# biscuitzb/COEB-SLAM

Hardware: AMD Instinct MI355X
Metric: frames/sec ORB extract+match @640x480/1000 kp; 1/2/4/8 GPU + %HBM roofline (higher is better)
Workload: dtype u8; 1 GPU; 640x480, 8-level pyramid, 1000 kp, extract + Hamming match to prev frame (BASELINE configs[1]); width=640, height=480, nfeatures=1000, nlevels=8, halo_frames_per_rank=1, pipelines_per_gpu=3, streams_per_gpu=1, ranks=single, parallelism=frame-sharded x1 (no collectives), hw_queues=4, side_stream=own, side_stream_created=with the context

## Files before the change

### coeb-slam_amd/csrc/coeb_extract.hip

```cpp
#include <type_traits>
#include <cmath>
#include <hip/hip_runtime.h>

#include "coeb_internal.hpp"

namespace {

constexpr int kThreads = 256;
constexpr int kWaves = kThreads / 64;

__device__ __forceinline__ int lane_id() { return __lane_id(); }
__device__ __forceinline__ int wave_id() { return __builtin_amdgcn_readfirstlane(threadIdx.x >> 6); }
__device__ __forceinline__ void wave_sync_lds()
{
    __builtin_amdgcn_fence(__ATOMIC_RELEASE, "wavefront");
    __builtin_amdgcn_wave_barrier();
    __builtin_amdgcn_fence(__ATOMIC_ACQUIRE, "wavefront");
}
typedef unsigned int u32x4 __attribute__((ext_vector_type(4)));

__device__ __forceinline__ uint64_t lanemask_lt() { return (1ull << lane_id()) - 1ull; }

__device__ __forceinline__ int wave_sum(int v)
{
// ... 81 lines not shown
        const int rx = (int)xmin, ry = (int)ymin, rw = (int)(xmax - xmin), rh = (int)(ymax - ymin);
        const float area_box = (xmax - xmin) * (ymax - ymin);
        bool mark = false;
        unsigned long long nin = 0;
        for (int t = t0; t < t1; t++) {
            const int px = (int)tm[2 * t], py = (int)tm[2 * t + 1];
            const bool in = px >= 0 && px < W && py >= 0 && py < H && px >= rx && px < rx + rw &&
                            py >= ry && py < ry + rh;
            if (in) nin++;
            if ((float)(nin * 10000ull) > area_box) { mark = true; break; }
        }
        const int bf = b.blurf ? b.blurf[bi] : 0;
        if (mark || (bf == 1 && nin > 0)) {
            area = area + area_box;
            const int x0 = max((int)xmin, 0), x1 = min((int)xmax, W);
            const int y0 = max((int)ymin, 0), y1 = min((int)ymax, H);
            if (x1 > x0 && y1 > y0) {
                if (m.nrect < COEB_MAXBOX) {
                    m.rect[m.nrect][0] = x0; m.rect[m.nrect][1] = y0;
                    m.rect[m.nrect][2] = x1; m.rect[m.nrect][3] = y1;
                    m.nrect++;
                } else {
                    atomicOr(b.err, 1);
                }
            }
        }
    }
    m.area_flag = area > 200000.f ? 1 : 0;
    b.dyn[f] = m;
}

typedef unsigned short us2 __attribute__((ext_vector_type(2)));
typedef float f32x2 __attribute__((ext_vector_type(2)));

__device__ __forceinline__ us2 as_us2(uint32_t v) { return __builtin_bit_cast(us2, v); }
__device__ __forceinline__ uint32_t as_u32(us2 v) { return __builtin_bit_cast(uint32_t, v); }
__device__ __forceinline__ us2 pk2(int lo, int hi) { us2 r; r.x = (unsigned short)lo; r.y = (unsigned short)hi; return r; }

__device__ __forceinline__ int byte_of(uint32_t w0, uint32_t w1, uint32_t w2, int o)
{
    const uint32_t w = o < 4 ? w0 : (o < 8 ? w1 : w2);
    return (int)((w >> ((o & 3) * 8)) & 0xFFu);
}

__device__ __forceinline__ uint32_t vresize_g(uint32_t g0, uint32_t g1, uint32_t b0s, uint32_t b1s)
{
    const uint32_t m0 = __umulhi(g0 & 0xFFFF00u, b0s & 0xFFFFFFu);
    const uint32_t m1 = __umulhi(g1 & 0xFFFF00u, b1s & 0xFFFFFFu);
    return (m0 + m1 + 2u) >> 2;
}

constexpr int PT_W = 128, PT_H = 32;

void pyr_tile_lds(int sw, int sh, int dw, int dh, int* tsw, int* tsh)
{
    const int span = (int)std::ceil(127.0 * sw / dw) + 2 + 15;
    *tsw = 16 * ((span + 15) / 16 + 1);
    *tsh = (int)std::ceil(31.0 * sh / dh) + 4;
}

int resize_simd_end(int w)
{
    int x = w >= 16 ? (w / 16) * 16 : 0;
    while (x < w - 4) x += 4;
    return x;
}

__device__ __forceinline__ uint32_t vresize_exact(uint32_t g0, uint32_t g1, uint32_t b0s, uint32_t b1s)
{
    const uint32_t v = __umul24(g0 >> 4, b0s >> 8) + __umul24(g1 >> 4, b1s >> 8) + (1u << 21);
    return min(v >> 22, 255u);
}

__global__ __launch_bounds__(kThreads) void k_pyr_level(const uint8_t* __restrict__ src, int64_t src_fs, int sp,
                                                        int sw, int sh, uint8_t* __restrict__ dst, int64_t dst_fs,
                                                        int dp, int dw, int dh, const int* __restrict__ tab, int xmax,
                                                        int xs, int tsw, int tsh)
{
    extern __shared__ __attribute__((aligned(16))) uint8_t s_src[];
    const int f = blockIdx.z;
    const int ox = blockIdx.x * PT_W, oy = blockIdx.y * PT_H;
    const int* xofs = tab;
    const int* alpha = tab + dw;
    const int* yofs = tab + 2 * dw;
    const int* beta = tab + 2 * dw + dh;
    const int ex = min(ox + PT_W, dw) - 1, ey = min(oy + PT_H, dh) - 1;
    const int sx1 = min(xofs[ex] + 1, sw - 1);
    const int sy0 = max(yofs[oy], 0), sy1 = min(max(yofs[ey] + 1, 0), sh - 1);
    const int nrows = sy1 - sy0 + 1;
    const uint8_t* S = src + (int64_t)f * src_fs;
    const int tid = threadIdx.x;
    int sx0;
    const bool vec = ((sp | (int)reinterpret_cast<uintptr_t>(S)) & 15) == 0;
    if (vec && ((sx1 - (xofs[ox] & ~15)) >> 4) + 1 <= tsw / 16 && nrows <= tsh) {
        sx0 = xofs[ox] & ~15;
        const int nch = ((sx1 - sx0) >> 4) + 1;
        const int rstep = kThreads / nch;
        const int r = tid / nch, k = tid - r * nch;
        if (r < rstep) {
            const uint4* base = reinterpret_cast<const uint4*>(S + (int64_t)sy0 * sp + sx0) + k;
            const int pw = sp >> 4;
            uint4 q0 = base[min(r, nrows - 1) * pw];
            uint4 q1 = base[min(r + rstep, nrows - 1) * pw];
            uint4 q2 = base[min(r + 2 * rstep, nrows - 1) * pw];
            if (r < nrows) *reinterpret_cast<uint4*>(s_src + r * tsw + 16 * k) = q0;
            if (r + rstep < nrows) *reinterpret_cast<uint4*>(s_src + (r + rstep) * tsw + 16 * k) = q1;
            if (r + 2 * rstep < nrows) *reinterpret_cast<uint4*>(s_src + (r + 2 * rstep) * tsw + 16 * k) = q2;
            for (int rr = r + 3 * rstep; rr < nrows; rr += rstep)
                *reinterpret_cast<uint4*>(s_src + rr * tsw + 16 * k) = base[rr * pw];
        }
    } else if ((sp & 3) == 0) {
        sx0 = xofs[ox] & ~3;
        const int nwords = (sx1 - sx0) / 4 + 1;
        for (int i = tid; i < nwords * nrows; i += kThreads) {
            const int r = i / nwords, k = i - r * nwords;
            *reinterpret_cast<uint32_t*>(s_src + r * tsw + 4 * k) =
                *reinterpret_cast<const uint32_t*>(S + (int64_t)(sy0 + r) * sp + sx0 + 4 * k);
        }
    } else {
        sx0 = xofs[ox];
        const int nb = sx1 - sx0 + 1;
        for (int i = tid; i < nb * nrows; i += kThreads) {
            const int r = i / nb, k = i - r * nb;
            s_src[r * tsw + k] = S[(int64_t)(sy0 + r) * sp + sx0 + k];
        }
    }
    __syncthreads();
    const int cx = ox + (threadIdx.x & 31) * 4, cy = oy + (threadIdx.x >> 5) * 4;
    if (cx >= dw) return;
    const int nk = min(4, dw - cx);
    int lx[4], a0[4], a1[4];
#pragma unroll
    for (int k = 0; k < 4; k++) {
        const int d = min(cx + k, dw - 1);
        const int sx = xofs[d];
        const int a = alpha[d];
        a0[k] = ((int)(short)(a & 0xFFFF)) << 4;
        a1[k] = (a >> 16) << 4;
        if (d >= xmax) { a0[k] = 2048 << 4; a1[k] = 0; }
        lx[k] = sx - sx0;
    }
#pragma unroll
    for (int r = 0; r < 4; r++) {
        const int dy = cy + r;
        if (dy >= dh) break;
        const int q0 = yofs[dy];
        const int r0 = (q0 >= 0 ? (q0 < sh ? q0 : sh - 1) : 0) - sy0;
        const int r1 = (q0 + 1 >= 0 ? (q0 + 1 < sh ? q0 + 1 : sh - 1) : 0) - sy0;
        const int bb = beta[dy];
        const uint32_t b0s = (uint32_t)((int)(short)(bb & 0xFFFF)) << 8, b1s = (uint32_t)(bb >> 16) << 8;
        const uint8_t* R0 = s_src + __mul24(r0, tsw);
        const uint8_t* R1 = s_src + __mul24(r1, tsw);
        uint32_t word = 0;
#pragma unroll
        for (int k = 0; k < 4; k++) {
            const int g0 = __mul24((int)R0[lx[k]], a0[k]) + __mul24((int)R0[lx[k] + 1], a1[k]);
            const int g1 = __mul24((int)R1[lx[k]], a0[k]) + __mul24((int)R1[lx[k] + 1], a1[k]);
            const uint32_t v = cx + k < xs ? vresize_g((uint32_t)g0, (uint32_t)g1, b0s, b1s)
                                           : vresize_exact((uint32_t)g0, (uint32_t)g1, b0s, b1s);
            word |= v << (8 * k);
        }
        uint8_t* D = dst + (int64_t)f * dst_fs + (int64_t)dy * dp + cx;
        if (nk == 4 && (dp & 3) == 0) *reinterpret_cast<uint32_t*>(D) = word;
        else for (int k = 0; k < nk; k++) D[k] = (uint8_t)(word >> (8 * k));
    }
}

constexpr int PR_ROWS = 8, PR_COLS = 128;

__device__ __forceinline__ uint32_t ld_u32(const uint8_t* p) { return *reinterpret_cast<const uint32_t*>(p); }

template <bool kTail, bool kEdge>
__device__ __forceinline__ void pyr_rows_out(const uint32_t (&w)[PR_ROWS][4], const uint32_t (&sel)[2],
                                             const uint32_t (&coef)[2], const int4* __restrict__ yrow,
                                             __amdgpu_buffer_rsrc_t rd, int oy, int dh, uint32_t cx, int dw, int xs)
{
#pragma unroll
    for (int r = 0; r < PR_ROWS; r++) {
        const int dy = oy + r;
        if (dy >= dh) break;
        const int4 yr = yrow[dy];
        const uint32_t bb = (uint32_t)yr.z;
        const uint32_t b0 = bb & 0xFFFFu, b1 = bb >> 16;
        const uint32_t b0s = (bb << 12) & 0xFFF000u, b1s = (bb >> 4) & 0xFFF000u;
        uint32_t v[2];
#pragma unroll
        for (int k = 0; k < 2; k++) {
            const uint32_t h0 = __builtin_amdgcn_udot2(as_us2(__builtin_amdgcn_perm(w[r][1], w[r][0], sel[k])),
                                                       as_us2(coef[k]), 0u, false);
            const uint32_t h1 = __builtin_amdgcn_udot2(as_us2(__builtin_amdgcn_perm(w[r][3], w[r][2], sel[k])),
                                                       as_us2(coef[k]), 0u, false);
            v[k] = (__umulhi(h0 & 0xFFFF0u, b0s) + __umulhi(h1 & 0xFFFF0u, b1s) + 2u) >> 2;
            if (kTail && (int)cx + k >= xs)
                v[k] = min((__umul24(h0, b0) + __umul24(h1, b1) + (1u << 21)) >> 22, 255u);
        }
        const uint32_t pr = v[0] | (v[1] << 8);
        if (!kEdge) {
            __builtin_amdgcn_raw_buffer_store_b16((uint16_t)pr, rd, cx, yr.w, 0);
        } else {
            if ((int)cx + 1 < dw) __builtin_amdgcn_raw_buffer_store_b16((uint16_t)pr, rd, cx, yr.w, 0);
            else if ((int)cx < dw) __builtin_amdgcn_raw_buffer_store_b8((uint8_t)pr, rd, cx, yr.w, 0);
        }
    }
}

__global__ __launch_bounds__(kThreads) void k_pyr_rows(const uint8_t* __restrict__ src, int64_t src_fs, int sp,
                                                       int sh, uint8_t* __restrict__ dst, int64_t dst_fs, int dp,
                                                       int dw, int dh, const int* __restrict__ tab, int xmax, int xs,
                                                       const int4* __restrict__ yrow)
{
    const int f = blockIdx.z;
    const int oy = (blockIdx.y * kWaves + wave_id()) * PR_ROWS;
    if (oy >= dh) return;
    const int lane = lane_id();
    const int ox = blockIdx.x * PR_COLS;
    const uint32_t cx = (uint32_t)(ox + 2 * lane);
    const int* xofs = tab;
    const int* alpha = tab + dw;
    uint32_t sel[2], coef[2];
    const int d0 = min((int)cx, dw - 1);
    const uint32_t wb = (uint32_t)(xofs[d0] & ~3);
    const uint32_t wb1 = (uint32_t)min((int)wb + 4, sp - 4);
#pragma unroll
    for (int k = 0; k < 2; k++) {
        const int d = min((int)cx + k, dw - 1);
        const int o = xofs[d] - (int)wb;
        const int a = alpha[d];
        const uint32_t a0 = d >= xmax ? 2048u : (uint32_t)(a & 0xFFFF), a1 = d >= xmax ? 0u : (uint32_t)a >> 16;
        coef[k] = a0 | (a1 << 16);
        sel[k] = (uint32_t)o | 0x0c00u | ((uint32_t)(o + 1) << 16) | 0x0c000000u;
    }
    const __amdgpu_buffer_rsrc_t rs =
        __builtin_amdgcn_make_buffer_rsrc((void*)(src + (int64_t)f * src_fs), 0, 0x7fffffff, 0x00020000);
    const __amdgpu_buffer_rsrc_t rd =
        __builtin_amdgcn_make_buffer_rsrc((void*)(dst + (int64_t)f * dst_fs), 0, 0x7fffffff, 0x00020000);
    uint32_t w[PR_ROWS][4];
#pragma unroll
    for (int r = 0; r < PR_ROWS; r++) {
        const int4 yr = yrow[min(oy + r, dh - 1)];
        w[r][0] = __builtin_amdgcn_raw_buffer_load_b32(rs, wb, yr.x, 0);
        w[r][1] = __builtin_amdgcn_raw_buffer_load_b32(rs, wb1, yr.x, 0);
        w[r][2] = __builtin_amdgcn_raw_buffer_load_b32(rs, wb, yr.y, 0);
        w[r][3] = __builtin_amdgcn_raw_buffer_load_b32(rs, wb1, yr.y, 0);
    }
    (void)dp;
    const bool edge = ox + PR_COLS > dw - 1;
    if (ox + PR_COLS > xs) {
        if (edge) pyr_rows_out<true, true>(w, sel, coef, yrow, rd, oy, dh, cx, dw, xs);
        else pyr_rows_out<true, false>(w, sel, coef, yrow, rd, oy, dh, cx, dw, xs);
    } else {
        if (edge) pyr_rows_out<false, true>(w, sel, coef, yrow, rd, oy, dh, cx, dw, xs);
        else pyr_rows_out<false, false>(w, sel, coef, yrow, rd, oy, dh, cx, dw, xs);
    }
}

constexpr int kBlurCols = 56;

__device__ __forceinline__ int reflect101(int p, int len)
{
    if (len == 1) return 0;
    while (p < 0 || p >= len) p = p < 0 ? -p : 2 * len - p - 2;
    return p;
}

struct BlurWork {
    int L;
    int item0, item1;
    int item_off[COEB_MAXL + 1];
    int nstrips[COEB_MAXL];
    int bh[COEB_MAXL];
    int nquads[COEB_MAXL];
    int brows;
};


template <bool kRemap = true>
__device__ __forceinline__ int2 block_xy()
{
    const int gx = gridDim.x;
    if (!kRemap) return make_int2(blockIdx.x, blockIdx.y);
    const int n = gx * gridDim.y, p = blockIdx.x + gx * blockIdx.y;
    const int q = n >> 3, r = n & 7, x = p & 7, k = p >> 3;
    const int lg = x * q + min(x, r) + k;
    return make_int2(lg % gx, lg / gx);
}

__device__ __forceinline__ uint32_t dpp_shr1(uint32_t v)
{
    return (uint32_t)__builtin_amdgcn_mov_dpp((int)v, 0x111, 0xf, 0xf, false);
}
__device__ __forceinline__ uint32_t dpp_shl1(uint32_t v)
{
    return (uint32_t)__builtin_amdgcn_mov_dpp((int)v, 0x101, 0xf, 0xf, false);
}

__device__ __forceinline__ int reflect_row(int r, int h)
{
    int rr = r < 0 ? -r : r;
    rr = rr >= h ? 2 * h - 2 - rr : rr;
    return rr < 0 ? 0 : rr;
}

constexpr int kBlurQuad = 4 * kBlurCols;
static_assert(kBlurQuad % 16 == 0, "a wave item must cover whole 16-column tiles");

__global__ __launch_bounds__(kThreads) void k_blur_rows(const Plan* __restrict__ P, ExtractBufs b, BlurWork bw)
{
    __shared__ __attribute__((aligned(16))) uint8_t s_tile[kWaves][8 * kBlurQuad];
    const int2 bxy = block_xy();
    const int f = bxy.y;
    const int item = bw.item0 + bxy.x * kWaves + wave_id();
    if (item >= bw.item1) return;
    int l = 0;
    while (l + 1 < bw.L && item >= bw.item_off[l + 1]) l++;
    const int it = item - bw.item_off[l];
    const int nq = bw.nquads[l];
    const int quad = it % nq, band = it / nq;
    const LevelGeom& g = P->lv[l];
    const int w = g.w, h = g.h, sp = g.pitch, dp = g.bpitch;
    const int lane = lane_id(), grp = lane >> 4, gl = lane & 15;
    const int y0 = band * bw.brows, y1 = min(h, y0 + bw.brows);
    const int x = (quad * 4 + grp) * kBlurCols - 4 + gl * 4;
    const bool produce = gl >= 1 && gl <= 14 && x < w;
    const int xbase = quad * kBlurQuad;
    uint8_t* tl = s_tile[wave_id()];
    int cq[4];
#pragma unroll
    for (int q = 0; q < 4; q++) cq[q] = reflect101(min(x + q, w + 2), w);
    const int a = min(min(min(cq[0], cq[1]), min(cq[2], cq[3])), w - 4);
    const uint32_t sel0 = 0x0c000c00u | (uint32_t)(cq[0] - a) | ((uint32_t)(cq[1] - a) << 16);
    const uint32_t sel1 = 0x0c000c00u | (uint32_t)(cq[2] - a) | ((uint32_t)(cq[3] - a) << 16);
    const __amdgpu_buffer_rsrc_t rs =
        __builtin_amdgcn_make_buffer_rsrc((void*)level_ptr(P, b, f, l), 0, 0x7fffffff, 0x00020000);
    const __amdgpu_buffer_rsrc_t rd =
        __builtin_amdgcn_make_buffer_rsrc((void*)(b.blur + (int64_t)f * P->blur_stride + g.blur_off), 0, 0x7fffffff,
                                          0x00020000);
    const int k0 = P->gauss[0], k1 = P->gauss[1], k2 = P->gauss[2], k3 = P->gauss[3];
    const us2 K0 = pk2(k0, k0), K1 = pk2(k1, k1), K2 = pk2(k2, k2), K3 = pk2(k3, k3);
    const us2 W_l01_0 = pk2(0, k0), W_l23_0 = pk2(k1, k2), W_c01_0 = pk2(k3, k2), W_c23_0 = pk2(k1, k0);
    const us2 W_l23_1 = pk2(k0, k1), W_c01_1 = pk2(k2, k3), W_c23_1 = pk2(k2, k1), W_r01_1 = pk2(k0, 0);
    const us2 W_l23_2 = pk2(0, k0), W_c01_2 = pk2(k1, k2), W_c23_2 = pk2(k3, k2), W_r01_2 = pk2(k1, k0);
    const us2 W_c01_3 = pk2(k0, k1), W_c23_3 = pk2(k2, k3), W_r01_3 = pk2(k2, k1), W_r23_3 = pk2(k0, 0);
    const uint32_t rnd = 1u << 15;
    const int n_rows = (y1 - y0) + 6;
    auto load_row = [&](int i) -> uint32_t {
        const int so = __builtin_amdgcn_readfirstlane(reflect_row(y0 - 3 + i, h) * sp);
        return __builtin_amdgcn_raw_buffer_load_b32(rs, a, so, 0);
    };
    uint32_t nxt[7];
#pragma unroll
    for (int ph = 0; ph < 7; ph++) nxt[ph] = load_row(ph);
    uint32_t R0[7], R1[7];
    for (int i0 = 0; i0 < n_rows; i0 += 7) {
        uint32_t raw[7];
#pragma unroll
        for (int ph = 0; ph < 7; ph++) raw[ph] = nxt[ph];
        if (i0 + 7 < n_rows) {
#pragma unroll
            for (int ph = 0; ph < 7; ph++) nxt[ph] = load_row(i0 + 7 + ph);
        }
#pragma unroll
        for (int ph = 0; ph < 7; ph++) {
            const int i = i0 + ph;
            if (i >= n_rows) break;
            R0[ph] = __builtin_amdgcn_perm(0u, raw[ph], sel0);
            R1[ph] = __builtin_amdgcn_perm(0u, raw[ph], sel1);
            if (i < 6) continue;
            const int s0 = (ph + 1) % 7, s1 = (ph + 2) % 7, s2 = (ph + 3) % 7, s3 = (ph + 4) % 7,
                      s4 = (ph + 5) % 7, s5 = (ph + 6) % 7, s6 = ph;
            const us2 v01 = K3 * as_us2(R0[s3]) + K2 * (as_us2(R0[s2]) + as_us2(R0[s4])) +
                            K1 * (as_us2(R0[s1]) + as_us2(R0[s5])) + K0 * (as_us2(R0[s0]) + as_us2(R0[s6]));
            const us2 v23 = K3 * as_us2(R1[s3]) + K2 * (as_us2(R1[s2]) + as_us2(R1[s4])) +
                            K1 * (as_us2(R1[s1]) + as_us2(R1[s5])) + K0 * (as_us2(R1[s0]) + as_us2(R1[s6]));
            const uint32_t V01 = as_u32(v01), V23 = as_u32(v23);
            const us2 L01 = as_us2(dpp_shr1(V01)), L23 = as_us2(dpp_shr1(V23));
            const us2 R01 = as_us2(dpp_shl1(V01)), R23 = as_us2(dpp_shl1(V23));
            uint32_t a0 = __builtin_amdgcn_udot2(L01, W_l01_0, rnd, false);
            a0 = __builtin_amdgcn_udot2(L23, W_l23_0, a0, false);
            a0 = __builtin_amdgcn_udot2(v01, W_c01_0, a0, false);
            a0 = __builtin_amdgcn_udot2(v23, W_c23_0, a0, false);
            uint32_t a1 = __builtin_amdgcn_udot2(L23, W_l23_1, rnd, false);
            a1 = __builtin_amdgcn_udot2(v01, W_c01_1, a1, false);
            a1 = __builtin_amdgcn_udot2(v23, W_c23_1, a1, false);
            a1 = __builtin_amdgcn_udot2(R01, W_r01_1, a1, false);
            uint32_t a2 = __builtin_amdgcn_udot2(L23, W_l23_2, rnd, false);
            a2 = __builtin_amdgcn_udot2(v01, W_c01_2, a2, false);
            a2 = __builtin_amdgcn_udot2(v23, W_c23_2, a2, false);
            a2 = __builtin_amdgcn_udot2(R01, W_r01_2, a2, false);
            uint32_t a3 = __builtin_amdgcn_udot2(v01, W_c01_3, rnd, false);
            a3 = __builtin_amdgcn_udot2(v23, W_c23_3, a3, false);
            a3 = __builtin_amdgcn_udot2(R01, W_r01_3, a3, false);
            a3 = __builtin_amdgcn_udot2(R23, W_r23_3, a3, false);
            const int y = y0 - 6 + i;
            if (produce) {
                const uint32_t p01 = __builtin_amdgcn_perm(a1, a0, 0x0c0c0602u);
                const uint32_t p23 = __builtin_amdgcn_perm(a3, a2, 0x06020c0cu);
                *reinterpret_cast<uint32_t*>(tl + (y & 7) * kBlurQuad + (x - xbase)) = p01 | p23;
            }
            if ((y & 7) == 7 || y == y1 - 1) {
                wave_sync_lds();
                const int so = __builtin_amdgcn_readfirstlane((int)blur_tile_off(0, y & ~7, dp));
#pragma unroll
                for (int k = 0; k < 2; k++) {
                    const int c = lane + 64 * k;
                    if (c < kBlurQuad / 2 && xbase + 16 * (c >> 3) < dp) {
                        const u32x4 v = *reinterpret_cast<const u32x4*>(tl + (c & 7) * kBlurQuad + 16 * (c >> 3));
                        __builtin_amdgcn_raw_buffer_store_b128(v, rd, (xbase >> 4) * 128 + 16 * c, so, 0);
                    }
                }
                wave_sync_lds();
            }
        }
    }
}

typedef const __attribute__((address_space(3))) uint8_t* lds_cu8;
typedef const __attribute__((address_space(3))) uint32_t* lds_cu32;

__device__ __forceinline__ void ring16(const uint8_t* c, int st, int p[16])
{
    p[0] = c[3 * st];      p[1] = c[3 * st + 1];  p[2] = c[2 * st + 2];  p[3] = c[st + 3];
    p[4] = c[3];           p[5] = c[-st + 3];     p[6] = c[-2 * st + 2]; p[7] = c[-3 * st + 1];
    p[8] = c[-3 * st];     p[9] = c[-3 * st - 1]; p[10] = c[-2 * st - 2]; p[11] = c[-st - 3];
    p[12] = c[-3];         p[13] = c[st - 3];     p[14] = c[2 * st - 2]; p[15] = c[3 * st - 1];
}

__device__ __forceinline__ int corner_strength(const uint8_t* c, int st)
{
    int p[16];
    ring16(c, st, p);
    const int v = c[0];
    int d[16];
#pragma unroll
    for (int k = 0; k < 16; k++) d[k] = v - p[k];
    int t[16];
#pragma unroll
    for (int k = 0; k < 16; k++) t[k] = min(min(d[k], d[(k + 1) & 15]), d[(k + 2) & 15]);
    int A = -1000;
#pragma unroll
    for (int k = 0; k < 16; k++) A = max(A, min(min(t[k], t[(k + 3) & 15]), t[(k + 6) & 15]));
#pragma unroll
    for (int k = 0; k < 16; k++) t[k] = max(max(d[k], d[(k + 1) & 15]), d[(k + 2) & 15]);
    int Bm = 1000;
#pragma unroll
    for (int k = 0; k < 16; k++) Bm = min(Bm, max(max(t[k], t[(k + 3) & 15]), t[(k + 6) & 15]));
    return max(A, -Bm);
}

constexpr int kFastRowBytes = 72;
constexpr int kFastRowBytesM = 96;
constexpr int kFastGuard = 16;
constexpr int kFastEnt = 128;
constexpr int kFastSurv = 4 * 64 + 8;
constexpr int kFastCorners = 256;
constexpr int kFastLists = kFastSurv;
static_assert(kFastRowBytesM * 64 <= 4 * 4096 && kFastRowBytes * 64 <= 4 * 4096, "k_fast entry offset field");


__device__ __forceinline__ bool fast_pretest(const uint8_t* c, int st, int t)
{
    const int v = c[0];
    const int lo = v - t, hi = v + t;
    auto cls = [&](int x) { return (x < lo ? 1 : 0) | (x > hi ? 2 : 0); };
    int d = cls(c[3 * st]) | cls(c[-3 * st]);
    d &= cls(c[2 * st + 2]) | cls(c[-2 * st - 2]);
    d &= cls(c[3]) | cls(c[-3]);
    d &= cls(c[-2 * st + 2]) | cls(c[2 * st - 2]);
    return d != 0;
}

__device__ __forceinline__ uint32_t win_lo(uint32_t a, uint32_t b, int s)
{
    return __builtin_amdgcn_perm(b, a, 0x0c000c00u | (uint32_t)s | ((uint32_t)(s + 1) << 16));
}
__device__ __forceinline__ uint32_t win_hi(uint32_t a, uint32_t b, int s)
{
    return __builtin_amdgcn_perm(b, a, 0x0c000c00u | (uint32_t)(s + 2) | ((uint32_t)(s + 3) << 16));
}

__device__ __forceinline__ us2 pk_min(us2 a, us2 b) { return __builtin_elementwise_min(a, b); }
__device__ __forceinline__ us2 pk_max(us2 a, us2 b) { return __builtin_elementwise_max(a, b); }
__device__ __forceinline__ us2 pk_subs(us2 a, us2 b) { return __builtin_elementwise_sub_sat(a, b); }

__device__ __forceinline__ us2 pk_max3(us2 a, us2 b, us2 c)
{
    uint32_t r;
    asm("v_pk_maximum3_f16 %0, %1, %2, %3" : "=v"(r) : "v"(as_u32(a)), "v"(as_u32(b)), "v"(as_u32(c)));
    return as_us2(r);
}
__device__ __forceinline__ us2 pk_min3(us2 a, us2 b, us2 c)
{
    uint32_t r;
    asm("v_pk_minimum3_f16 %0, %1, %2, %3" : "=v"(r) : "v"(as_u32(a)), "v"(as_u32(b)), "v"(as_u32(c)));
    return as_us2(r);
}

__device__ __forceinline__ uint32_t pretest_half(us2 v, us2 p0, us2 p8, us2 p2, us2 p10, us2 p4, us2 p12, us2 p6,
                                                 us2 p14, us2 T)
{
    const us2 md = pk_max3(pk_min(p0, p8), pk_min(p2, p10), pk_max(pk_min(p4, p12), pk_min(p6, p14)));
    const us2 mb = pk_min3(pk_max(p0, p8), pk_max(p2, p10), pk_min(pk_max(p4, p12), pk_max(p6, p14)));
    return as_u32(pk_subs(pk_max(pk_subs(v, md), pk_subs(mb, v)), T));
}

template <bool kMax, bool S1, bool S2>
__device__ __forceinline__ uint32_t pk3(uint32_t a, uint32_t b, uint32_t c)
{
    uint32_t r;
#define COEB_PK3(OP, SEL) asm(OP " %0, %1, %2, %3" SEL : "=v"(r) : "v"(a), "v"(b), "v"(c))
    if constexpr (kMax) {
        if constexpr (!S1 && !S2) COEB_PK3("v_pk_maximum3_f16", "");
        else if constexpr (!S1 && S2) COEB_PK3("v_pk_maximum3_f16", " op_sel:[0,0,1] op_sel_hi:[1,1,0]");
        else if constexpr (S1 && !S2) COEB_PK3("v_pk_maximum3_f16", " op_sel:[0,1,0] op_sel_hi:[1,0,1]");
        else COEB_PK3("v_pk_maximum3_f16", " op_sel:[0,1,1] op_sel_hi:[1,0,0]");
    } else {
        if constexpr (!S1 && !S2) COEB_PK3("v_pk_minimum3_f16", "");
        else if constexpr (!S1 && S2) COEB_PK3("v_pk_minimum3_f16", " op_sel:[0,0,1] op_sel_hi:[1,1,0]");
        else if constexpr (S1 && !S2) COEB_PK3("v_pk_minimum3_f16", " op_sel:[0,1,0] op_sel_hi:[1,0,1]");
        else COEB_PK3("v_pk_minimum3_f16", " op_sel:[0,1,1] op_sel_hi:[1,0,0]");
    }
#undef COEB_PK3
    return r;
}

__device__ __forceinline__ uint32_t arc_max_min_pk(const uint32_t Q[8])
{
    uint32_t M3[8], M9[8];
#pragma unroll
    for (int k = 0; k < 6; k++) M3[k] = pk3<false, false, false>(Q[k], Q[k + 1], Q[k + 2]);
    M3[6] = pk3<false, false, true>(Q[6], Q[7], Q[0]);
    M3[7] = pk3<false, true, true>(Q[7], Q[0], Q[1]);
    M9[0] = pk3<false, false, false>(M3[0], M3[3], M3[6]);
    M9[1] = pk3<false, false, false>(M3[1], M3[4], M3[7]);
#pragma unroll
    for (int k = 2; k < 5; k++) M9[k] = pk3<false, false, true>(M3[k], M3[k + 3], M3[k - 2]);
#pragma unroll
    for (int k = 5; k < 8; k++) M9[k] = pk3<false, true, true>(M3[k], M3[k - 5], M3[k - 2]);
    const uint32_t A = pk3<true, false, false>(M9[0], M9[1], M9[2]);
    const uint32_t B = pk3<true, false, false>(M9[3], M9[4], M9[5]);
    return pk3<true, false, false>(M9[6], M9[7], pk3<true, false, false>(A, B, A));
}

template <int st>
__device__ __forceinline__ int corner_strength_pos2(const uint8_t* c, int t)
{
    lds_cu8 b = (lds_cu8)c - (3 * st + 1);
    asm volatile("" : "+v"(b));
    constexpr int o = 3 * st + 1;
    constexpr int off[16] = {o + 3 * st, o + 3 * st + 1, o + 2 * st + 2, o + st + 3, o + 3, o - st + 3, o - 2 * st + 2,
                             o - 3 * st + 1, 1, 0, o - 2 * st - 2, o - st - 3, o - 3, o + st - 3, o + 2 * st - 2,
                             o + 3 * st - 1};
    us2 Qv[8];
#pragma unroll
    for (int k = 0; k < 8; k++) { Qv[k].x = b[off[k]]; Qv[k].y = b[off[k + 8]]; }
    const int v = b[o];
    uint32_t Q[8];
#pragma unroll
    for (int k = 0; k < 8; k++) Q[k] = as_u32(Qv[k]);
    auto lo = [](uint32_t x) { return (int)(x & 0xFFFFu); };
    auto hi = [](uint32_t x) { return (int)(x >> 16); };
    const int md = max(max(min(lo(Q[0]), hi(Q[0])), min(lo(Q[2]), hi(Q[2]))),
                       max(min(lo(Q[4]), hi(Q[4])), min(lo(Q[6]), hi(Q[6]))));
    const int mb = min(min(max(lo(Q[0]), hi(Q[0])), max(lo(Q[2]), hi(Q[2]))),
                       min(max(lo(Q[4]), hi(Q[4])), max(lo(Q[6]), hi(Q[6]))));
    const bool dark = md < v - t, bright = mb > v + t;
    const uint32_t mask = dark ? 0x00FF00FFu : 0u;
    uint32_t Qx[8];
#pragma unroll
    for (int k = 0; k < 8; k++) Qx[k] = Q[k] ^ mask;
    const uint32_t X = arc_max_min_pk(Qx);
    int M = max(lo(X), hi(X)) - (v ^ (int)(mask & 0xFFu));
    if (__builtin_expect(__ballot(dark && bright) != 0, 0)) {
        if (dark && bright) {
            const uint32_t Y = arc_max_min_pk(Q);
            M = max(M, max(lo(Y), hi(Y)) - v);
        }
    }
    return M;
}

template <int RB>
__device__ __forceinline__ void fast_pretest4_raw(const uint8_t* c, int t, uint32_t& lo, uint32_t& hi)
{
    constexpr int st = RB;
    lds_cu32 w = (lds_cu32)(c - 3 * st);
    asm volatile("" : "+v"(w));
    constexpr int o = 3 * st / 4;
    const uint32_t a0 = w[o - 1], b0 = w[o], c0 = w[o + 1];
    const uint32_t ap = w[o + 2 * st / 4 - 1], bp = w[o + 2 * st / 4], cp = w[o + 2 * st / 4 + 1];
    const uint32_t am = w[o - 2 * st / 4 - 1], bm = w[o - 2 * st / 4], cm = w[o - 2 * st / 4 + 1];
    const uint32_t u3 = w[o + 3 * st / 4];
    const uint32_t d3 = w[0];
    const us2 T = pk2(t, t);
    lo = pretest_half(
        as_us2(__builtin_amdgcn_perm(0u, b0, 0x0c010c00u)), as_us2(__builtin_amdgcn_perm(0u, u3, 0x0c010c00u)),
        as_us2(__builtin_amdgcn_perm(0u, d3, 0x0c010c00u)), as_us2(win_lo(bp, cp, 2)), as_us2(win_lo(am, bm, 2)),
        as_us2(win_lo(b0, c0, 3)), as_us2(win_lo(a0, b0, 1)), as_us2(win_lo(bm, cm, 2)), as_us2(win_lo(ap, bp, 2)), T);
    hi = pretest_half(
        as_us2(__builtin_amdgcn_perm(0u, b0, 0x0c030c02u)), as_us2(__builtin_amdgcn_perm(0u, u3, 0x0c030c02u)),
        as_us2(__builtin_amdgcn_perm(0u, d3, 0x0c030c02u)), as_us2(win_hi(bp, cp, 2)), as_us2(win_hi(am, bm, 2)),
        as_us2(win_hi(b0, c0, 3)), as_us2(win_hi(a0, b0, 1)), as_us2(win_hi(bm, cm, 2)), as_us2(win_hi(ap, bp, 2)), T);
}

template <int RB>
__device__ __forceinline__ int fast_mi(int o, int mp)
{
    if constexpr (RB == kFastRowBytesM) {
        return o + 45;
    } else {
        const int yy = (int)((unsigned)o / (unsigned)RB);
        return (yy - 2) * mp + (o - yy * RB) - 3;
    }
}

__device__ __forceinline__ int nms_keep(const uint8_t* Ms, int mi, int mp, int t, int* sc_out)
{
    const int M = Ms[mi];
    if (M <= t) return 0;
    const int sc = M - 1;
    bool kept = true;
#pragma unroll
    for (int dy = -1; dy <= 1; dy++)
#pragma unroll
        for (int dx = -1; dx <= 1; dx++) {
            if (dx == 0 && dy == 0) continue;
            const int Mn = Ms[mi + dy * mp + dx];
            const int ns = Mn > t ? Mn - 1 : 0;
            kept = kept && (sc > ns);
        }
    *sc_out = sc;
    return kept ? 1 : 0;
}

__device__ __forceinline__ int mbcnt(uint64_t m)
{
    return (int)__builtin_amdgcn_mbcnt_hi((uint32_t)(m >> 32), __builtin_amdgcn_mbcnt_lo((uint32_t)m, 0u));
}
__device__ __forceinline__ int uniform(int v) { return __builtin_amdgcn_readfirstlane(v); }

constexpr int kFastPass = 12;

struct FastCellGeom {
    const uint8_t* img;
    int pitch, x0, y0, rw, rh, nwords;
    bool vec;
    bool words;
};

struct FastRegs {
    u32x4 v0, v1, v2;
};

__device__ __forceinline__ FastCellGeom fast_geom(const Plan* P, const ExtractBufs& b, int f, const CellDesc& c)
{
    FastCellGeom G;
    const LevelGeom& g = P->lv[c.level];
    G.img = level_ptr(P, b, f, c.level);
    G.pitch = g.pitch;
    G.x0 = c.x0; G.y0 = c.y0; G.rw = c.rw; G.rh = c.rh;
    G.nwords = (1 + c.rw + 3) >> 2;
    G.vec = ((g.pitch | (int)reinterpret_cast<uintptr_t>(G.img)) & 15) == 0 && G.nwords <= 12 && c.rh <= 48;
    G.words = (g.pitch & 3) == 0 && G.nwords <= 15 && c.rh <= 4 * kFastPass;
    return G;
}

__device__ __forceinline__ void fast_prefetch(const FastCellGeom& G, FastRegs& R)
{
    const int lane = lane_id();
    if (G.vec) {
        const uint8_t* base = G.img + (int64_t)G.y0 * G.pitch + ((G.x0 - 1) & ~15) + 16 * (lane & 3);
        const int r = lane >> 2;
        R.v0 = *reinterpret_cast<const u32x4*>(base + (int64_t)min(r, G.rh - 1) * G.pitch);
        R.v1 = *reinterpret_cast<const u32x4*>(base + (int64_t)min(r + 16, G.rh - 1) * G.pitch);
        R.v2 = *reinterpret_cast<const u32x4*>(base + (int64_t)min(r + 32, G.rh - 1) * G.pitch);
    }
}

__device__ __attribute__((aligned(64))) const uint8_t g_fast_zero[64] = {0};

__device__ __forceinline__ void fast_dma(const FastCellGeom& G, uint8_t* roi)
{
    typedef __attribute__((address_space(3))) void* lds_vp;
    const int lane = lane_id();
    const int nq = 6 * G.rh;
    const uint8_t* row0 = G.img + (int64_t)G.y0 * G.pitch + (G.x0 - 1);
#pragma unroll
    for (int i = 0; i < 5; i++) {
        if (64 * i < nq) {
            const int q = 64 * i + lane;
            const int r = (q * 171) >> 10;
            const int k = q - 6 * r;
            const uint8_t* src = k < 3 ? row0 + r * G.pitch + 16 * k : g_fast_zero;
            if (q < nq) __builtin_amdgcn_global_load_lds((const void*)src, (lds_vp)(roi + 1024 * i), 16, 0, 0);
        }
    }
}
__device__ __forceinline__ void fast_dma_wait() { asm volatile("s_waitcnt vmcnt(0)" ::: "memory"); }

template <int RB>
__device__ __forceinline__ void fast_stage(const FastCellGeom& G, const FastRegs& R, uint8_t* roi)
{
    const int lane = lane_id();
    if (G.vec) {
        const int sh = (G.x0 - 1) & 15;
        const int r = lane >> 2, c = lane & 3;
        uint8_t* d = roi + r * RB + 16 * c - sh;
        if (r < G.rh) __builtin_memcpy(d, &R.v0, 16);
        if (r + 16 < G.rh) __builtin_memcpy(d + 16 * RB, &R.v1, 16);
        if (r + 32 < G.rh) __builtin_memcpy(d + 32 * RB, &R.v2, 16);
        if constexpr (RB == kFastRowBytesM) {
            asm volatile("" ::: "memory");
            uint8_t* z = roi + r * RB + 48 + 16 * c;
            const uint4 zero = make_uint4(0, 0, 0, 0);
            if (c < 3 && r < G.rh) *reinterpret_cast<uint4*>(z) = zero;
            if (c < 3 && r + 16 < G.rh) *reinterpret_cast<uint4*>(z + 16 * RB) = zero;
            if (c < 3 && r + 32 < G.rh) *reinterpret_cast<uint4*>(z + 32 * RB) = zero;
// ... 1388 lines not shown
```

Before: 380,300 frames/s.

## Restructure row-blur loop into 8-row blocks with padded LDS tile and reflect-free fast path

Reworks the vertical/horizontal blur kernel's row loop so rows are processed in 8-row blocks aligned with the 8-row output tile, removing per-row branch checks for the flush condition and the modulo-7 ring indexing. It adds an interior-band specialization that replaces per-row reflect_row computation with a linear offset increment, pads the LDS tile pitch by 16 bytes to reduce bank conflicts, and precomputes store addresses and predicates outside the loop. Non-producing lanes write to a dummy padding slot instead of branching. The change adds code size and register pressure from two template instantiations.

```diff
diff --git a/coeb-slam_amd/csrc/coeb_extract.hip b/coeb-slam_amd/csrc/coeb_extract.hip
--- a/coeb-slam_amd/csrc/coeb_extract.hip
+++ b/coeb-slam_amd/csrc/coeb_extract.hip
@@ -407,11 +407,12 @@
 }
 
 constexpr int kBlurQuad = 4 * kBlurCols;
+constexpr int kBlurPitch = kBlurQuad + 16;
 static_assert(kBlurQuad % 16 == 0, "a wave item must cover whole 16-column tiles");
 
 __global__ __launch_bounds__(kThreads) void k_blur_rows(const Plan* __restrict__ P, ExtractBufs b, BlurWork bw)
 {
-    __shared__ __attribute__((aligned(16))) uint8_t s_tile[kWaves][8 * kBlurQuad];
+    __shared__ __attribute__((aligned(16))) uint8_t s_tile[kWaves][8 * kBlurPitch];
     const int2 bxy = block_xy();
     const int f = bxy.y;
     const int item = bw.item0 + bxy.x * kWaves + wave_id();
@@ -447,76 +448,122 @@
     const us2 W_l23_2 = pk2(0, k0), W_c01_2 = pk2(k1, k2), W_c23_2 = pk2(k3, k2), W_r01_2 = pk2(k1, k0);
     const us2 W_c01_3 = pk2(k0, k1), W_c23_3 = pk2(k2, k3), W_r01_3 = pk2(k2, k1), W_r23_3 = pk2(k0, 0);
     const uint32_t rnd = 1u << 15;
-    const int n_rows = (y1 - y0) + 6;
-    auto load_row = [&](int i) -> uint32_t {
-        const int so = __builtin_amdgcn_readfirstlane(reflect_row(y0 - 3 + i, h) * sp);
-        return __builtin_amdgcn_raw_buffer_load_b32(rs, a, so, 0);
+    const int nfull = (y1 - y0) >> 3, tail = (y1 - y0) & 7;
+    uint32_t R0[8], R1[8];
+    auto take = [&](int s, uint32_t raw) {
+        R0[s] = __builtin_amdgcn_perm(0u, raw, sel0);
+        R1[s] = __builtin_amdgcn_perm(0u, raw, sel1);
     };
-    uint32_t nxt[7];
-#pragma unroll
-    for (int ph = 0; ph < 7; ph++) nxt[ph] = load_row(ph);
-    uint32_t R0[7], R1[7];
-    for (int i0 = 0; i0 < n_rows; i0 += 7) {
-        uint32_t raw[7];
-#pragma unroll
-        for (int ph = 0; ph < 7; ph++) raw[ph] = nxt[ph];
-        if (i0 + 7 < n_rows) {
-#pragma unroll
-            for (int ph = 0; ph < 7; ph++) nxt[ph] = load_row(i0 + 7 + ph);
-        }
-#pragma unroll
-        for (int ph = 0; ph < 7; ph++) {
-            const int i = i0 + ph;
-            if (i >= n_rows) break;
-            R0[ph] = __builtin_amdgcn_perm(0u, raw[ph], sel0);
-            R1[ph] = __builtin_amdgcn_perm(0u, raw[ph], sel1);
-            if (i < 6) continue;
-            const int s0 = (ph + 1) % 7, s1 = (ph + 2) % 7, s2 = (ph + 3) % 7, s3 = (ph + 4) % 7,
-                      s4 = (ph + 5) % 7, s5 = (ph + 6) % 7, s6 = ph;
-            const us2 v01 = K3 * as_us2(R0[s3]) + K2 * (as_us2(R0[s2]) + as_us2(R0[s4])) +
-                            K1 * (as_us2(R0[s1]) + as_us2(R0[s5])) + K0 * (as_us2(R0[s0]) + as_us2(R0[s6]));
-            const us2 v23 = K3 * as_us2(R1[s3]) + K2 * (as_us2(R1[s2]) + as_us2(R1[s4])) +
-                            K1 * (as_us2(R1[s1]) + as_us2(R1[s5])) + K0 * (as_us2(R1[s0]) + as_us2(R1[s6]));
-            const uint32_t V01 = as_u32(v01), V23 = as_u32(v23);
-            const us2 L01 = as_us2(dpp_shr1(V01)), L23 = as_us2(dpp_shr1(V23));
-            const us2 R01 = as_us2(dpp_shl1(V01)), R23 = as_us2(dpp_shl1(V23));
-            uint32_t a0 = __builtin_amdgcn_udot2(L01, W_l01_0, rnd, false);
-            a0 = __builtin_amdgcn_udot2(L23, W_l23_0, a0, false);
-            a0 = __builtin_amdgcn_udot2(v01, W_c01_0, a0, false);
-            a0 = __builtin_amdgcn_udot2(v23, W_c23_0, a0, false);
-            uint32_t a1 = __builtin_amdgcn_udot2(L23, W_l23_1, rnd, false);
-            a1 = __builtin_amdgcn_udot2(v01, W_c01_1, a1, false);
-            a1 = __builtin_amdgcn_udot2(v23, W_c23_1, a1, false);
-            a1 = __builtin_amdgcn_udot2(R01, W_r01_1, a1, false);
-            uint32_t a2 = __builtin_amdgcn_udot2(L23, W_l23_2, rnd, false);
-            a2 = __builtin_amdgcn_udot2(v01, W_c01_2, a2, false);
-            a2 = __builtin_amdgcn_udot2(v23, W_c23_2, a2, false);
-            a2 = __builtin_amdgcn_udot2(R01, W_r01_2, a2, false);
-            uint32_t a3 = __builtin_amdgcn_udot2(v01, W_c01_3, rnd, false);
-            a3 = __builtin_amdgcn_udot2(v23, W_c23_3, a3, false);
-            a3 = __builtin_amdgcn_udot2(R01, W_r01_3, a3, false);
-            a3 = __builtin_amdgcn_udot2(R23, W_r23_3, a3, false);
-            const int y = y0 - 6 + i;
-            if (produce) {
-                const uint32_t p01 = __builtin_amdgcn_perm(a1, a0, 0x0c0c0602u);
-                const uint32_t p23 = __builtin_amdgcn_perm(a3, a2, 0x06020c0cu);
-                *reinterpret_cast<uint32_t*>(tl + (y & 7) * kBlurQuad + (x - xbase)) = p01 | p23;
-            }
-            if ((y & 7) == 7 || y == y1 - 1) {
-                wave_sync_lds();
-                const int so = __builtin_amdgcn_readfirstlane((int)blur_tile_off(0, y & ~7, dp));
-#pragma unroll
-                for (int k = 0; k < 2; k++) {
-                    const int c = lane + 64 * k;
-                    if (c < kBlurQuad / 2 && xbase + 16 * (c >> 3) < dp) {
-                        const u32x4 v = *reinterpret_cast<const u32x4*>(tl + (c & 7) * kBlurQuad + 16 * (c >> 3));
-                        __builtin_amdgcn_raw_buffer_store_b128(v, rd, (xbase >> 4) * 128 + 16 * c, so, 0);
-                    }
-                }
-                wave_sync_lds();
-            }
-        }
-    }
+    typedef __attribute__((address_space(3))) uint32_t* lds_u32;
+    lds_u32 trow = (lds_u32)(tl + (produce ? x - xbase : kBlurQuad + 8 * (grp & 1) + 4 * (gl & 1)));
+    asm volatile("" : "+v"(trow));
+    auto out_row = [&](int s, int k) {
+        const int s0 = (s + 2) & 7, s1 = (s + 3) & 7, s2 = (s + 4) & 7, s3 = (s + 5) & 7, s4 = (s + 6) & 7,
+                  s5 = (s + 7) & 7, s6 = s;
+        const us2 v01 = K3 * as_us2(R0[s3]) + K2 * (as_us2(R0[s2]) + as_us2(R0[s4])) +
+                        K1 * (as_us2(R0[s1]) + as_us2(R0[s5])) + K0 * (as_us2(R0[s0]) + as_us2(R0[s6]));
+        const us2 v23 = K3 * as_us2(R1[s3]) + K2 * (as_us2(R1[s2]) + as_us2(R1[s4])) +
+                        K1 * (as_us2(R1[s1]) + as_us2(R1[s5])) + K0 * (as_us2(R1[s0]) + as_us2(R1[s6]));
+        const uint32_t V01 = as_u32(v01), V23 = as_u32(v23);
+        const us2 L01 = as_us2(dpp_shr1(V01)), L23 = as_us2(dpp_shr1(V23));
+        const us2 R01 = as_us2(dpp_shl1(V01)), R23 = as_us2(dpp_shl1(V23));
+        uint32_t a0 = __builtin_amdgcn_udot2(L01, W_l01_0, rnd, false);
+        a0 = __builtin_amdgcn_udot2(L23, W_l23_0, a0, false);
+        a0 = __builtin_amdgcn_udot2(v01, W_c01_0, a0, false);
+        a0 = __builtin_amdgcn_udot2(v23, W_c23_0, a0, false);
+        uint32_t a1 = __builtin_amdgcn_udot2(L23, W_l23_1, rnd, false);
+        a1 = __builtin_amdgcn_udot2(v01, W_c01_1, a1, false);
+        a1 = __builtin_amdgcn_udot2(v23, W_c23_1, a1, false);
+        a1 = __builtin_amdgcn_udot2(R01, W_r01_1, a1, false);
+        uint32_t a2 = __builtin_amdgcn_udot2(L23, W_l23_2, rnd, false);
+        a2 = __builtin_amdgcn_udot2(v01, W_c01_2, a2, false);
+        a2 = __builtin_amdgcn_udot2(v23, W_c23_2, a2, false);
+        a2 = __builtin_amdgcn_udot2(R01, W_r01_2, a2, false);
+        uint32_t a3 = __builtin_amdgcn_udot2(v01, W_c01_3, rnd, false);
+        a3 = __builtin_amdgcn_udot2(v23, W_c23_3, a3, false);
+        a3 = __builtin_amdgcn_udot2(R01, W_r01_3, a3, false);
+        a3 = __builtin_amdgcn_udot2(R23, W_r23_3, a3, false);
+        const uint32_t p01 = __builtin_amdgcn_perm(a1, a0, 0x0c0c0602u);
+        const uint32_t p23 = __builtin_amdgcn_perm(a3, a2, 0x06020c0cu);
+        trow[k * (kBlurPitch / 4)] = p01 | p23;
+    };
+    const int c1 = lane + 64;
+    const bool st0 = xbase + 16 * (lane >> 3) < dp;
+    const bool st1 = c1 < kBlurQuad / 2 && xbase + 16 * (c1 >> 3) < dp;
+    const uint8_t* const tsrc0 = tl + (lane & 7) * kBlurPitch + 16 * (lane >> 3);
+    const uint8_t* const tsrc1 = tl + (c1 & 7) * kBlurPitch + 16 * (c1 >> 3);
+    const int tdst = (xbase >> 4) * 128 + 16 * lane;
+    int so_d = __builtin_amdgcn_readfirstlane((int)blur_tile_off(0, y0, dp));
+    const int so_dstep = __builtin_amdgcn_readfirstlane((dp >> 4) * 128);
+    auto flush = [&]() {
+        wave_sync_lds();
+        if (st0) __builtin_amdgcn_raw_buffer_store_b128(*reinterpret_cast<const u32x4*>(tsrc0), rd, tdst, so_d, 0);
+        if (st1)
+            __builtin_amdgcn_raw_buffer_store_b128(*reinterpret_cast<const u32x4*>(tsrc1), rd, tdst + 16 * 64, so_d, 0);
+        wave_sync_lds();
+        so_d += so_dstep;
+    };
+    auto band_rows = [&](auto reflect) {
+        constexpr bool kReflect = decltype(reflect)::value;
+        int r = y0 - 3;
+        int so = __builtin_amdgcn_readfirstlane((y0 - 3) * sp);
+        auto load_row = [&]() -> uint32_t {
+            int o;
+            if constexpr (kReflect) {
+                o = __builtin_amdgcn_readfirstlane(reflect_row(r, h) * sp);
+                r++;
+            } else {
+                o = so;
+                so += sp;
+            }
+            return __builtin_amdgcn_raw_buffer_load_b32(rs, a, o, 0);
+        };
+        uint32_t pro[6], nxt[8];
+#pragma unroll
+        for (int s = 0; s < 6; s++) pro[s] = load_row();
+#pragma unroll
+        for (int k = 0; k < 8; k++) nxt[k] = 0u;
+        if (nfull > 0) {
+#pragma unroll
+            for (int k = 0; k < 8; k++) nxt[k] = load_row();
+        } else {
+#pragma unroll
+            for (int k = 0; k < 7; k++)
+                if (k < tail) nxt[k] = load_row();
+        }
+#pragma unroll
+        for (int s = 0; s < 6; s++) take(s, pro[s]);
+        for (int blk = 0; blk < nfull; blk++) {
+            uint32_t raw[8];
+#pragma unroll
+            for (int k = 0; k < 8; k++) raw[k] = nxt[k];
+            if (blk + 1 < nfull) {
+#pragma unroll
+                for (int k = 0; k < 8; k++) nxt[k] = load_row();
+            } else {
+#pragma unroll
+                for (int k = 0; k < 7; k++)
+                    if (k < tail) nxt[k] = load_row();
+            }
+#pragma unroll
+            for (int k = 0; k < 8; k++) {
+                take((6 + k) & 7, raw[k]);
+                out_row((6 + k) & 7, k);
+            }
+            flush();
+        }
+        if (tail) {
+#pragma unroll
+            for (int k = 0; k < 7; k++) {
+                if (k >= tail) break;
+                take((6 + k) & 7, nxt[k]);
+                out_row((6 + k) & 7, k);
+            }
+            flush();
+        }
+    };
+    if (y0 >= 3 && y1 + 2 < h) band_rows(std::false_type());
+    else band_rows(std::true_type());
 }
 
 typedef const __attribute__((address_space(3))) uint8_t* lds_cu8;
```

Measured after the change: 385,600 frames/s (median of 6 runs). 1.01x the previous value.
